# wexiangis/wmix

Measured on AMD Instinct MI355X. Metric: 10 ms frames/s, higher is better.
Workload: dtype f32

## Files before the change

### tools_dev/aec_prof.py

```python
import sys, ctypes; sys.path.insert(0,'.')
import numpy as np, torch
from wmix_amd import synth, _lib
from wmix_amd.aec import AecBatch
dev=torch.device('cuda:0'); S=int(sys.argv[1]) if len(sys.argv)>1 else 65536
import os
if os.environ.get('WMX_TOOL_LIB'): _lib.LIB_PATH=os.environ['WMX_TOOL_LIB']
lib=_lib.lib(); f=lib.wmx_debug_aec_prof; f.argtypes=[ctypes.c_void_p,ctypes.c_int]
ab=AecBatch(S,1,16000,10); nf=24
far=synth.far_end(5,nf,160); near=synth.near_end(50,64,nf,160,far=far)
dfar=torch.from_numpy(far.reshape(nf,160).copy()).to(dev)
dn=torch.from_numpy(np.ascontiguousarray(near.reshape(64,nf,160).transpose(1,0,2))).to(dev).repeat(1,S//64,1).contiguous()
buf=(ctypes.c_ulonglong*16)()
for k in range(nf):
    if k==16: f(buf,1)
    ab.process2_packet_major(dfar[k:k+1],dn[k:k+1])
f(buf,0); v=np.array(buf[:16],dtype=np.float64)
names=['near ring+d,dw fft','dpow+filterfar','y ifft+e,ew fft','scale+adapt','partdelay','xfw+psd','sd/se sums','coh+hNl+scalars','overdrive+cn','ifft+ola','state in','(all pkts)','state out','scale_err','pack','24 ffts']
tot=v[10]+v[12]+v[11]
for n,x in zip(names,v): print('%-20s %8.1f Mcyc %5.1f%%'%(n,x/1e6,100*x/tot))
print('pcm io etc', (v[11]-v[:10].sum()-v[13:].sum())/1e6)
```

### tools_dev/ns_prof.py

```python
import sys, ctypes; sys.path.insert(0,'.')
import numpy as np, torch
from wmix_amd import synth, _lib
from wmix_amd.ns import NsBatch
dev=torch.device('cuda:0'); S=int(sys.argv[1]) if len(sys.argv)>1 else 65536
import os
if os.environ.get('WMX_TOOL_LIB'): _lib.LIB_PATH=os.environ['WMX_TOOL_LIB']
lib=_lib.lib(); f=lib.wmx_debug_ns_prof; f.argtypes=[ctypes.c_void_p,ctypes.c_int]
nb=NsBatch(S,1,16000); nf=int(sys.argv[2]) if len(sys.argv)>2 else 260
x=synth.ns_input(7,64,nf,160)
d=torch.from_numpy(np.ascontiguousarray(x.reshape(64,nf,160).transpose(1,0,2))).to(dev).repeat(1,S//64,1).contiguous()
buf=(ctypes.c_ulonglong*16)()
for k in range(nf):
    if k==nf-8: f(buf,1)
    nb.process_packet_major(d[k:k+1])
f(buf,0); v=np.array(buf[:14],dtype=np.float64)
names=['load+window+energy1','fft fwd','spectrum+log','7 sums','noise est (quantiles)','startup/snr loop','3 sums+flat','lrt loop (log)','ksum+prior+exp loop','noise update+wiener','ifft','td+energy2','synth+hb','output']
for n,x in zip(names,v): print('%-24s %8.1f Mcyc %5.1f%%'%(n,x/1e6,100*x/v.sum()))
```

### wmix_amd/csrc/aec.hip

```cpp
#include <algorithm>
#include <chrono>
#include <cmath>
#include <cstdlib>
#include <cstring>
#include <cstddef>
#include <unordered_map>
#include <vector>
#include "wmx_internal.h"
#include "aec_ctl.h"
#include "cohort_hip.h"
#include "fft_regs.h"
#include "libm_dev.h"

namespace wmx {
namespace {

constexpr int BP = 68;
enum : int {
    AS_W_RE = 0,
    AS_W_IM = AS_W_RE + 12 * BP,
    AS_DPOW = AS_W_IM + 12 * BP,
    AS_DMIN = AS_DPOW + BP,
    AS_DINIT = AS_DMIN + BP,
    AS_SD = AS_DINIT + BP,
// ... 303 lines not shown
    int16_t park[kAecFrame];
#ifdef WMX_AEC_PROF
    unsigned long long prof[16];
#endif
};
#define AEC_ST(x) W.st[(x) - AS_LDS0]

struct AecTaps {
    v2f t[12];
};

__device__ __forceinline__ float uniform_ld(const float *p) {
    return *reinterpret_cast<const float __attribute__((address_space(4))) *>(reinterpret_cast<size_t>(p));
}

typedef const float __attribute__((address_space(1))) *GlobalRow;
__device__ __forceinline__ GlobalRow uniform_row(const float *base, int row, int row_words) {
    const float *p = base + (size_t)row * row_words;
    asm volatile("" : "+s"(p));
    return (GlobalRow)p;
}

__device__ __forceinline__ float row_ld(GlobalRow row, unsigned lane_bytes, int word) {
    return *(GlobalRow)((const char __attribute__((address_space(1))) *)(row + word) + lane_bytes);
}

constexpr int kHistRowBytes = 130 * 4, kHistMid = 2860;
struct HistRows {
    GlobalRow base;
    unsigned voff;
// ... 12 lines not shown

__device__ __forceinline__ int ring_at(int pos, int i) {
    const int t = pos + i;
    return t >= kAecRing ? t - kAecRing : t;
}
__device__ __forceinline__ float *fa_row(AecWaveLds &W, int r) { return &W.fa[0][0] + __umul24((unsigned)r, (unsigned)FAS); }
__device__ __forceinline__ int opaque_lane(int x) {
#ifndef WMX_AEC_HOIST
    asm volatile("" : "+v"(x));
#endif
    __builtin_assume(x >= 0 && x < 64);
    return x;
}

template <int MULT>
__device__ __forceinline__ void aec_block(const AecConstsNear &K, const float *__restrict__ curves_g, const PowTables *__restrict__ powtab, AecWaveLds &W, AecTaps &taps,
                                          const AecFarBufs &F, const AecBlkPlan &bp, const AecNoiseEntry *__restrict__ noise_tab, const int lane_in) {
    int lane = opaque_lane(lane_in);
    int *Si = reinterpret_cast<int *>(W.st) - AS_LDS0;
    const float mu = MULT == 1 ? 0.6f : 0.5f, err_thr = MULT == 1 ? 2e-6f : 1.5e-6f;
    const float scale = 2.0f / 128;
    const int n = bp.hist_n;
    int blk_flags;
    {
        int nctr = __builtin_amdgcn_readfirstlane(Si[AS_NOISECTR]), dctr = __builtin_amdgcn_readfirstlane(Si[AS_DELAYCTR]);
        blk_flags = nctr > 50 ? kAecFlagNoiseMin : 0;
        if (nctr < 500 * MULT) {
            nctr++;
            blk_flags |= kAecFlagNoiseInit;
        }
        dctr++;
        if (dctr == 10 * MULT) dctr = 0;
// ... 359 lines not shown
    const int diverge = ((Si[AS_DIVERGE] ? 1.05f : 1.0f) * seSum > sdSum) ? 1 : 0;
    const bool reset_filter = seSum > (19.95f * sdSum);
    wave_sync();
    if (lane == 0) Si[AS_DIVERGE] = diverge;
    if (reset_filter) {
#pragma unroll
        for (int p = 0; p < 12; p++) {
            taps.t[p] = v2f{0.f, 0.f};
            if (lane == 0) W.wn[p] = 0.f;
        }
    }
    AEC_PROF(6);
    AEC_RELANE();
    const uint32_t nseed = (uint32_t)__builtin_amdgcn_readfirstlane(Si[AS_NSEED]);
    const uint2 *jump = reinterpret_cast<const uint2 *>(noise_tab + kAecNoiseTab);
    const uint2 jl = jump[(lane + 63) & 63], j64 = jump[63];
    const AecNoiseEntry nz = noise_tab[((nseed * jl.x + jl.y) & 0x7FFFFFFFu) >> 16];
    const float nz_c = nz.c, nz_s = nz.s;
    if (lane == 0) Si[AS_NSEED] = (int)((nseed * j64.x + j64.y) & 0x7FFFFFFFu);
    {
        auto coh = [&](int b, float &cde, float &cxd) {
            const float sde_r = AEC_ST(AS_SDE_RE + b), sde_i = AEC_ST(AS_SDE_IM + b), sxd_r = AEC_ST(AS_SXD_RE + b),
                        sxd_i = AEC_ST(AS_SXD_IM + b);
            cde = (sde_r * sde_r + sde_i * sde_i) / (AEC_ST(AS_SD + b) * AEC_ST(AS_SE + b) + 1e-10f);
            cxd = (sxd_r * sxd_r + sxd_i * sxd_i) / (AEC_ST(AS_SX + b) * AEC_ST(AS_SD + b) + 1e-10f);
        };
        float a0, a1, c0, c1;
        coh(lane, a0, a1);
#if !defined(WMX_AEC_EXP) || WMX_AEC_EXP < 1
        coh(kAecPart, c0, c1);
#else
// ... 172 lines not shown
            AEC_ST(AS_OUT_RING + ring_at(bp.out_wr, i + 1)) = o1;
        }
        wave_sync();
        if (lane >= 32) {
            AEC_ST(AS_OUTBUF + i) = pt.x * scale * K.hanning[kAecPart - i];
            AEC_ST(AS_OUTBUF + i + 1) = pt.y * scale * K.hanning[kAecPart - i - 1];
        }
    }
    AEC_ST(AS_DPREV + lane) = W.cur[lane];
    AEC_ST(AS_EPREV + lane) = W.enew[lane];
    wave_sync();
    AEC_PROF(9);
#undef AEC_RELANE
}

template <int MULT>
#ifndef WMX_AEC_WAVES
#define WMX_AEC_WAVES 4
#endif
__global__ __attribute__((amdgpu_waves_per_eu(WMX_AEC_WAVES, WMX_AEC_WAVES))) __launch_bounds__(64 * kAecWavesPerBlock) void aec_near_kernel(float *__restrict__ state, AecFarBufs F_all,
                                                                          const float *__restrict__ consts_g,
                                                                          const AecPlan *__restrict__ plans, int n_packets, int n_classes,
                                                                          const int32_t *__restrict__ plan_of,
                                                                          const AecNoiseEntry *__restrict__ noise_tab,
                                                                          const int16_t *near_pcm, int16_t *out_pcm, int n_streams,
                                                                          long stream_stride, long packet_stride, int chn, int pkg,
                                                                          const int *__restrict__ stream_far, const uint8_t *__restrict__ active,
                                                                          const int *__restrict__ order) {
    __shared__ AecConstsNear K;
    __shared__ AecWaveLds Wv[kAecWavesPerBlock];
    const int lane = threadIdx.x & 63;
    const int wave = __builtin_amdgcn_readfirstlane(threadIdx.x >> 6);
    int sidx;
    if (order) {
        const unsigned i = blockIdx.x, per = gridDim.x >> 3;
        sidx = __builtin_amdgcn_readfirstlane(order[((i & 7u) * per + (i >> 3)) * kAecWavesPerBlock + wave]);
    } else {
        sidx = blockIdx.x * kAecWavesPerBlock + wave;
    }
    const bool live = sidx >= 0 && stream_active(active, sidx, n_streams);
    const int sl = (sidx >= 0 && sidx < n_streams) ? sidx : 0;
    const int grp = stream_far ? __builtin_amdgcn_readfirstlane(stream_far[sl]) : 0;
    const AecFarBufs F = far_group(F_all, grp);
    plans += plan_of ? __builtin_amdgcn_readfirstlane(plan_of[grp]) : grp;
    float *gst = state + (size_t)sl * AS_WORDS;
    constexpr int kConstIt = (kAecConstNearWords + 64 * kAecWavesPerBlock - 1) / (64 * kAecWavesPerBlock);
    float kc[kConstIt];
#pragma unroll
    for (int k = 0; k < kConstIt; k++) {
        const int i = threadIdx.x + 64 * kAecWavesPerBlock * k;
        kc[k] = consts_g[i < kAecConstNearWords ? i : 0];
    }
    int16_t pcm0[2][2];
    {
        const int16_t *in0 = near_pcm + (size_t)sl * stream_stride;
#pragma unroll
        for (int s = 0; s < 2; s++)
#pragma unroll
            for (int h = 0; h < 2; h++) {
                const int i = lane + 64 * h;
                const bool want = i < kAecFrame && s * kAecFrame + i < pkg;
                const int16_t v = in0[want ? (s * kAecFrame + i) * chn : 0];
                pcm0[s][h] = want ? v : (int16_t)0;
            }
    }
    AecTaps taps;
#pragma unroll
    for (int p = 0; p < 12; p++) {
        taps.t[p].x = gst[AS_W_RE + p * BP + lane];
        taps.t[p].y = gst[AS_W_IM + p * BP + lane];
    }
    const float wn0 = gst[AS_W_RE + (lane < 12 ? lane : 0) * BP + kAecPart];
    constexpr int kChunks = (AS_LDS_WORDS / 4 + 63) / 64;
    float4 c[kChunks];
    {
        const float4 *g4 = reinterpret_cast<const float4 *>(gst + AS_LDS0);
#pragma unroll
        for (int k = 0; k < kChunks; k++) {
            const int i = lane + 64 * k;
            c[k] = g4[i < AS_LDS_WORDS / 4 ? i : i - 64];
        }
    }
#pragma unroll
    for (int k = 0; k < kConstIt; k++) {
        const int i = threadIdx.x + 64 * kAecWavesPerBlock * k;
        if (i < kAecConstNearWords) reinterpret_cast<float *>(&K)[i] = kc[k];
    }
    asm volatile("s_waitcnt lgkmcnt(0)\n\ts_barrier" ::: "memory");
    if (!live) return;
    const PowTables *powtab = reinterpret_cast<const PowTables *>(consts_g + kAecConstWords);
    AecWaveLds &W = Wv[wave];
#ifdef WMX_AEC_PROF
    if (lane < 16) W.prof[lane] = 0;
#endif
    AEC_PROF_START;
    if (lane < 12) W.wn[lane] = wn0;
    {
        float4 *s4 = reinterpret_cast<float4 *>(W.st);
#pragma unroll
        for (int k = 0; k < kChunks; k++) {
            const int i = lane + 64 * k;
            s4[i < AS_LDS_WORDS / 4 ? i : i - 64] = c[k];
        }
    }
#pragma unroll
    for (int h = 0; h < 2; h++) {
        const int i = lane + 64 * h;
        if (i < kAecFrame) {
            W.fa[0][i] = (float)pcm0[0][h];
            W.park[i] = pcm0[1][h];
        }
    }
    wave_sync();
    AEC_PROF(10);
    for (int p = 0; p < n_packets; p++) {
        const AecPlan &pl = plans[(size_t)p * n_classes];
        if (!pl.has_near) continue;
        const size_t off = (size_t)sidx * stream_stride + (size_t)p * packet_stride;
        const int16_t *in = near_pcm + off;
        int16_t *out = out_pcm + off;
        if (pl.passthrough) {
            for (int i = lane; i < pkg; i += 64) {
                const int16_t v = in[i * chn];
                for (int c = 0; c < chn; c++) out[i * chn + c] = v;
            }
            continue;
        }
        for (int s = 0; s < pl.n_sub; s++) {
            const AecSubPlan &sp = pl.sub[s];
            const int ln = opaque_lane(lane);
#pragma unroll
            for (int h = 0; h < 2; h++) {
                const int i = ln + 64 * h;
                if (i >= kAecFrame) continue;
                const float v = (p == 0 && s < 2) ? (s == 0 ? W.fa[0][i] : (float)W.park[i]) : (float)in[(s * kAecFrame + i) * chn];
                AEC_ST(AS_NEAR_RING + ring_at(sp.near_wr, i)) = v;
            }
            wave_sync();
            for (int k = 0; k < sp.n_blocks; k++)
                aec_block<MULT>(K, consts_g + kAecConstNearWords, powtab, W, taps, F, pl.blk[sp.first_blk + k], noise_tab, lane);
            for (int i = opaque_lane(lane); i < kAecFrame; i += 64) {
                const int16_t v = (int16_t)AEC_ST(AS_OUT_RING + ring_at(sp.out_rd, i));
                for (int c = 0; c < chn; c++) out[(s * kAecFrame + i) * chn + c] = v;
            }
            wave_sync();
        }
    }
    wave_sync();
    AEC_PROF(11);
    asm volatile("" : "+s"(gst));
    float __attribute__((address_space(1))) *gout = (float __attribute__((address_space(1))) *)gst;
    const int ln = opaque_lane(lane);
#pragma unroll
    for (int p = 0; p < 12; p++) {
        gout[AS_W_RE + p * BP + ln] = taps.t[p].x;
        gout[AS_W_IM + p * BP + ln] = taps.t[p].y;
    }
    if (ln < 12) gout[AS_W_RE + ln * BP + kAecPart] = W.wn[ln];
    {
        typedef float v4f __attribute__((ext_vector_type(4)));
        v4f __attribute__((address_space(1))) *g4 = (v4f __attribute__((address_space(1))) *)(gout + AS_LDS0);
        const v4f *s4 = reinterpret_cast<const v4f *>(W.st);
        for (int i = ln; i < AS_LDS_WORDS / 4; i += 64) g4[i] = s4[i];
    }
    AEC_PROF(12);
#ifdef WMX_AEC_PROF
    if (lane < 16) atomicAdd(&g_aec_prof[lane], W.prof[lane]);
#endif
}
#ifdef WMX_AEC_PROF
extern "C" int wmx_debug_aec_prof(unsigned long long *out16, int reset) {
    hipDeviceSynchronize();
    hipMemcpyFromSymbol(out16, HIP_SYMBOL(g_aec_prof), sizeof(unsigned long long) * 16);
    if (reset) {
        unsigned long long z[16] = {0};
        hipMemcpyToSymbol(HIP_SYMBOL(g_aec_prof), z, sizeof(z));
    }
    return 0;
}
#endif


// ... 82 lines not shown
    wmx::AecFarBufs far;
    int *d_stream_far;
    std::vector<int32_t> h_cohort_of;
    std::vector<int32_t> h_order[2];
    int h_order_sel;
    int32_t *d_order;
    unsigned order_wgs;
    bool order_dirty;
    int order_age;
    static constexpr int kOrderEvery = 16;
    wmx::AecNoiseEntry *d_noise_tab;
    wmx::StreamLife life;
    bool timing;
    std::vector<hipEvent_t> tev;
    size_t tev_used;
    bool no_order;
    double ctl_seconds;
    long ctl_calls;
    static constexpr size_t kMaxTimingEvents = 4 * 4096;
};

extern "C" {

int wmx_aec_destroy(wmx_aec *h) {
    WMX_ON_DEVICE(h);
    if (!h) return 0;
    if (h->d_state) (void)hipFree(h->d_state);
    if (h->d_consts) (void)hipFree(h->d_consts);
    if (h->d_stream_far) (void)hipFree(h->d_stream_far);
    if (h->d_order) (void)hipFree(h->d_order);
// ... 134 lines not shown
    std::vector<float> st(AS_WORDS, 0.f);
    for (int b = 0; b < 65; b++) {
        st[AS_DMIN + b] = 1.0e6f;
        st[AS_SD + b] = 1.f;
        st[AS_SX + b] = 1.f;
    }
    st[AS_HNLFBMIN] = 1.f;
    st[AS_HNLFBLOCALMIN] = 1.f;
    st[AS_HNLXDAVGMIN] = 1.f;
    st[AS_OVERDRIVE] = 2.f;
    st[AS_OVERDRIVESM] = 2.f;
    {
        const uint32_t seed0 = 777u;
        memcpy(&st[AS_NSEED], &seed0, 4);
    }
    WMX_CREATE_TRY(wmx_aec_destroy(h), hipMalloc(&h->d_state, (size_t)AS_WORDS * n_streams * sizeof(float)));
    WMX_CREATE_TRY(wmx_aec_destroy(h), hipMalloc(&h->d_consts, sizeof(K) + sizeof(PowTables)));
    for (hipEvent_t &ev : h->co.plan_free) WMX_CREATE_TRY(wmx_aec_destroy(h), hipEventCreateWithFlags(&ev, hipEventDisableTiming));
    {
        const int rc = h->co.reserve(n_far, [h] { aec_carve_far(h); });
        if (rc != 0) {
            wmx_aec_destroy(h);
            return rc;
        }
    }
    if (n_far > 1) {
        WMX_CREATE_TRY(wmx_aec_destroy(h), hipMalloc(&h->d_stream_far, sizeof(int) * n_streams));
        if (stream_far) {
            WMX_CREATE_TRY(wmx_aec_destroy(h), hipMemcpy(h->d_stream_far, stream_far, sizeof(int) * n_streams, hipMemcpyHostToDevice));
        } else {
// ... 127 lines not shown
            WMX_HIP(hipEventRecord(tv[0], fs));
        }
        hipLaunchKernelGGL(aec_far_kernel, dim3((unsigned)L.G), dim3(64), 0, fs, h->far, h->d_consts, L.dp, L.chunk, L.C, L.plan_of,
                           d_far ? d_far + (size_t)L.done * far_packet_stride : nullptr, far_packet_stride, far_group_stride, h->chn, gpow1np,
                           L.by_value, L.hp[0]);
        WMX_LAUNCH_CHECK();
        if (tv) WMX_HIP(hipEventRecord(tv[1], fs));
        return 0;
    };
    auto near = [&](const CohortLaunch<AecPlan> &L) {
        if (tv) WMX_HIP(hipEventRecord(tv[2], s));
        const int16_t *nin = d_near + (size_t)L.done * packet_stride;
        int16_t *nout = d_out + (size_t)L.done * packet_stride;
        if (h->order_age < wmx_aec::kOrderEvery) h->order_age++;
        const int32_t *order = ordered ? h->d_order : nullptr;
        const unsigned grid = ordered ? h->order_wgs : (unsigned)((h->n_streams + kAecWavesPerBlock - 1) / kAecWavesPerBlock);
        const dim3 blk(64 * kAecWavesPerBlock);
        if (h->freq == 8000)
            hipLaunchKernelGGL((aec_near_kernel<1>), dim3(grid), blk, 0, s, h->d_state, h->far, h->d_consts, L.dp, L.chunk, L.C, L.plan_of,
                               h->d_noise_tab, nin, nout, h->n_streams, stream_stride, packet_stride, h->chn, h->pkg, h->d_stream_far,
                               h->life.d_active, order);
        else
            hipLaunchKernelGGL((aec_near_kernel<2>), dim3(grid), blk, 0, s, h->d_state, h->far, h->d_consts, L.dp, L.chunk, L.C, L.plan_of,
                               h->d_noise_tab, nin, nout, h->n_streams, stream_stride, packet_stride, h->chn, h->pkg, h->d_stream_far,
                               h->life.d_active, order);
        WMX_LAUNCH_CHECK();
        if (tv) WMX_HIP(hipEventRecord(tv[3], s));
        return 0;
    };
    return run_cohorts(h, "wmx_aec_run", mode, d_far, far_packet_stride, far_group_stride, d_near, d_out, n_packets, stream_stride,
                       packet_stride, delay_ms, cohort_on, cohort_rc, s, before, plan, far, near);
}

int wmx_aec_reset_streams(wmx_aec *h, const int32_t *idx, int n, int cohort, void *stream) {
    using namespace wmx;
    int refused = 0;
    if (h && (cohort < -1 || cohort >= h->co.n()))
        refused = WMX_EINVAL;
    else if (h && cohort >= 0 && h->co.n() > 1 && !h->d_stream_far)
        refused = WMX_ESTATE;
// ... 145 lines not shown
```

### wmix_amd/csrc/ns.hip

```cpp
#include <cmath>
#include <vector>
#include "stage_life.h"
#include "fft_ooura.h"
#include "libm_dev.h"
#include "ns_layout.h"

namespace wmx {
namespace {

constexpr int kStartupShort = 50;
constexpr int kStartupLong = 200;
constexpr int kHistBins = 1000;
constexpr int kUpdateWindow = 500;
constexpr int kStartBand = 5;

constexpr int kNsWavesPerBlock = 4;

template <int L>
struct NsConstLds {
    FftTables tab;
    float window[L];
    float logi[NsLayout<L>::MP];
    NsLibmTables lm;
};
// ... 57 lines not shown
        if (i + 1 < MP4) {
            const float4 b = *reinterpret_cast<const float4 *>(mine + 4 * i + 4);
            acc += b.x;
            acc += b.y;
            acc += b.z;
            acc += b.w;
        }
    }
    return acc;
}
__device__ __noinline__ static float tanh_call(float x, const NsLibmTables *m) { return fast_tanh(x, *m); }
__device__ __forceinline__ float lane_value(float v, int k) { return __int_as_float(__builtin_amdgcn_readlane(__float_as_int(v), k)); }

template <int L, int CHN>
__device__ void ns_frame(const NsConstLds<L> &K, NsWaveLds<L> &W, float *__restrict__ st, unsigned short *__restrict__ hist,
                         const int16_t *in, int16_t *out, const int pkg, const int lane_in) {
    using Y = NsLayout<L>;
    constexpr int chn = CHN;
    int lane = lane_in;
#define NS_RELANE() asm volatile("" : "+v"(lane))
    NS_RELANE();
#ifdef WMX_NS_PROF
    long long prof_t0 = clock64();
#endif
    constexpr int M = Y::M, B = Y::B, NT = L / 64, NC = L / 2;
    struct StF {
        GlobalF g;
        unsigned i;
        __device__ __forceinline__ operator float() const { return row_ld(g, i); }
        __device__ __forceinline__ void operator=(float v) const { row_st(g, i, v); }
    };
// ... 36 lines not shown
#else
    constexpr int NI = (M + 63) / 64;
#endif
    float pf_quant[NI], pf_dens[NI][3], pf_lq[NI][3], pf_pause[NI];
#pragma unroll
    for (int k = 0; k < NI; k++) {
        const int b = lane + 64 * k < M ? lane + 64 * k : M - 1;
        pf_pause[k] = ST(Y::MAGN_AVG_PAUSE + b);
        pf_quant[k] = ST(Y::QUANTILE + b);
#pragma unroll
        for (int q = 0; q < 3; q++) {
            pf_dens[k][q] = ST(Y::DENSITY + q * Y::MP + b);
            pf_lq[k][q] = ST(Y::LQUANTILE + q * Y::MP + b);
        }
    }
    wave_sync();
#pragma unroll
    for (int k = 0; k < NT; k++) {
        const int i = lane + 64 * k;
        if (64 * k + 63 < B) continue;
        if (i >= B) {
            ST(Y::IN_BUF + i) = buf[k];
            if (chn == 2) ST(Y::HB_BUF + i) = hb[k];
        }
    }
#pragma unroll
    for (int k = 0; k < NT; k++) {
        const int i = lane + 64 * k;
        const float w = K.window[i] * buf[k];
        W.fa[i] = w;
        tdst[i] = w * w;
    }
    wave_sync();
    const float energy1 = sum_range(tdst, 0, L, lane);
    wave_sync();
    NS_PROF(0);

    float hb_gain = 1.f;
    const bool zero_frame = (energy1 == 0.0f);
    float t_re[(Y::M + 63) / 64], t_im[(Y::M + 63) / 64], t_prev[(Y::M + 63) / 64], t_snrq[(Y::M + 63) / 64];

    if (!zero_frame) {
        const int block_ind = SCI(S_BLOCK_IND) + 1;
        STI(Y::S_BLOCK_IND) = block_ind;
        const int update_flag = SCI(S_UPDATE_FLAG);
        const bool startup = block_ind < kStartupShort;
        const float overdrive = 1.1f, denoise_bound = 0.125f;

        NS_RELANE();
        rdft_forward<NC>(W.fa, &K.tab, lane);
        if (lane < Y::MP - M) W.r0[M + lane] = 0.f;
// ... 457 lines not shown
            ST(Y::MAGN_PREV + b) = mg;
            ST(Y::NOISE_PREV + b) = nz;
            W.snrp[b] = f;
            if (b == 0)
                W.fa[0] = re;
            else if (b == M - 1)
                W.fa[1] = re;
            else {
                W.fa[2 * b] = re;
                W.fa[2 * b + 1] = im;
            }
        }
        wave_sync();
        NS_PROF(9);
        NS_RELANE();
        rdft_inverse<NC>(W.fa, &K.tab, lane);
        NS_PROF(10);
        float td[NT];
#pragma unroll
        for (int k = 0; k < NT; k++) {
            const int i = lane + 64 * k;
            td[k] = W.fa[i] * (2.f / L);
            tdst[i] = td[k] * td[k];
        }
        wave_sync();
        NS_PROF(11);
        float factor = 1.f;
        if (block_ind > kStartupLong) {
            const float energy2 = sum_range(tdst, 0, L, lane);
            float gain = sqrtf(energy2 / (energy1 + 1.f));
// ... 59 lines not shown

#ifndef WMX_NS_W128
#define WMX_NS_W128 7
#endif
#ifndef WMX_NS_W256
#define WMX_NS_W256 5
#endif
template <int L>
struct NsOcc {
    static constexpr int kWaves = L == 128 ? WMX_NS_W128 : WMX_NS_W256;
};
template <int L, int CHN>
__global__ __launch_bounds__(64 * kNsWavesPerBlock) __attribute__((amdgpu_waves_per_eu(NsOcc<L>::kWaves, NsOcc<L>::kWaves))) void ns_kernel(float *__restrict__ state, unsigned short *__restrict__ hists,
                                                                      const float *__restrict__ consts, const int16_t *in, int16_t *out,
                                                                      int n_streams, int n_packets, long stream_stride,
                                                                      long packet_stride, int pkg, const uint8_t *__restrict__ active) {
    using Y = NsLayout<L>;
    __shared__ NsConstLds<L> K;
    __shared__ NsWaveLds<L> Wv[kNsWavesPerBlock];
    {
        float *dst = reinterpret_cast<float *>(&K);
        constexpr int NCONST = sizeof(NsConstLds<L>) / 4, NIT = (NCONST + 64 * kNsWavesPerBlock - 1) / (64 * kNsWavesPerBlock);
        float c[NIT];
#pragma unroll
        for (int k = 0; k < NIT; k++) {
            const int i = threadIdx.x + 64 * kNsWavesPerBlock * k;
            c[k] = consts[i < NCONST ? i : 0];
        }
#pragma unroll
        for (int k = 0; k < NIT; k++) {
            const int i = threadIdx.x + 64 * kNsWavesPerBlock * k;
            if (i < NCONST) dst[i] = c[k];
        }
    }
    __syncthreads();
    const int lane = threadIdx.x & 63;
    const int wave = __builtin_amdgcn_readfirstlane(threadIdx.x >> 6);
    const int sidx = blockIdx.x * kNsWavesPerBlock + wave;
    if (!stream_active(active, sidx, n_streams)) return;
    float *st = state + (size_t)sidx * Y::WORDS;
    unsigned short *hist = hists + (size_t)sidx * 3 * kHistBins;
    {
        float *wb = Wv[wave].magn;
        constexpr int NARR = 9;
        if (lane < NARR * (Y::MP - Y::M)) wb[(lane / (Y::MP - Y::M)) * Y::MP + Y::M + lane % (Y::MP - Y::M)] = 0.f;
    }
#ifdef WMX_NS_PROF
    if (lane < 16) Wv[wave].prof[lane] = 0;
#endif
    for (int p = 0; p < n_packets; p++) {
        const size_t off = (size_t)sidx * stream_stride + (size_t)p * packet_stride;
        ns_frame<L, CHN>(K, Wv[wave], st, hist, in + off, out + off, pkg, lane);
    }
#ifdef WMX_NS_PROF
    if (lane < 16) atomicAdd(&g_ns_prof[lane], Wv[wave].prof[lane]);
#endif
}
#ifdef WMX_NS_PROF
extern "C" int wmx_debug_ns_prof(unsigned long long *out16, int reset) {
    (void)hipDeviceSynchronize();
    (void)hipMemcpyFromSymbol(out16, HIP_SYMBOL(g_ns_prof), sizeof(unsigned long long) * 16);
    if (reset) {
        unsigned long long z[16] = {0};
        (void)hipMemcpyToSymbol(HIP_SYMBOL(g_ns_prof), z, sizeof(z));
    }
    return 0;
}
#endif

}
}

struct wmx_ns {
    int device;
    int n_streams, chn, freq, L, pkg;
    float *d_state;
    unsigned short *d_hist;
    float *d_consts;
    float *d_tmpl;
    size_t words;
    wmx::StreamLife life;
};

namespace {

template <int L>
void build_ns_template(std::vector<float> &st, std::vector<float> &consts) {
    using Y = wmx::NsLayout<L>;
    st.assign(Y::WORDS, 0.f);
    int *sti = reinterpret_cast<int *>(st.data());
    for (int q = 0; q < 3; q++)
        for (int b = 0; b < Y::M; b++) {
            st[Y::LQUANTILE + q * Y::MP + b] = 8.f;
            st[Y::DENSITY + q * Y::MP + b] = 0.3f;
        }
// ... 63 lines not shown
    if ((h->device = wmx::current_device()) < 0) {
        delete h;
        return WMX_ENODEV;
    }
    h->n_streams = n_streams;
    h->chn = chn;
    h->freq = freq;
    h->L = (freq == 8000) ? 128 : 256;
    h->pkg = freq / 1000 * 10;
    std::vector<float> st, consts;
    if (h->L == 128)
        build_ns_template<128>(st, consts);
    else
        build_ns_template<256>(st, consts);
    h->words = st.size();
    WMX_CREATE_TRY(wmx_ns_destroy(h), hipMalloc(&h->d_state, h->words * sizeof(float) * (size_t)n_streams));
    WMX_CREATE_TRY(wmx_ns_destroy(h), hipMalloc(&h->d_hist, (size_t)n_streams * 3 * 1000 * sizeof(unsigned short)));
    WMX_CREATE_TRY(wmx_ns_destroy(h), hipMalloc(&h->d_consts, consts.size() * sizeof(float)));
    WMX_CREATE_TRY(wmx_ns_destroy(h), hipMalloc(&h->d_tmpl, st.size() * sizeof(float)));
    WMX_CREATE_TRY(wmx_ns_destroy(h), hipMemcpy(h->d_consts, consts.data(), consts.size() * sizeof(float), hipMemcpyHostToDevice));
    WMX_CREATE_TRY(wmx_ns_destroy(h), hipMemcpy(h->d_tmpl, st.data(), st.size() * sizeof(float), hipMemcpyHostToDevice));
    WMX_CREATE_TRY(wmx_ns_destroy(h), hipMemset(h->d_hist, 0, (size_t)n_streams * 3 * 1000 * sizeof(unsigned short)));
    hipLaunchKernelGGL(ns_fill_state, dim3(1024), dim3(256), 0, nullptr, h->d_state, h->d_tmpl, (int)h->words, n_streams);
    WMX_CREATE_TRY(wmx_ns_destroy(h), hipGetLastError());
    WMX_CREATE_TRY(wmx_ns_destroy(h), hipDeviceSynchronize());
    *out = h;
    return 0;
}

int wmx_ns_destroy(wmx_ns *h) {
// ... 46 lines not shown
    WMX_ON_DEVICE(h);
    if (!h || n_packets < 0) {
        wmx::set_error("wmx_ns_process: bad argument");
        return WMX_EINVAL;
    }
    if (n_packets == 0) return 0;
    if (!d_in || !d_out) {
        wmx::set_error("wmx_ns_process: null buffer");
        return WMX_EINVAL;
    }
    const int per_pkt = h->pkg * h->chn;
    if (packet_stride < per_pkt || (h->n_streams > 1 && stream_stride < per_pkt)) {
        wmx::set_error("wmx_ns_process: strides (%ld, %ld) smaller than a packet (%d samples)", stream_stride, packet_stride, per_pkt);
        return WMX_EINVAL;
    }
    const unsigned grid = (unsigned)((h->n_streams + wmx::kNsWavesPerBlock - 1) / wmx::kNsWavesPerBlock);
    hipStream_t s = wmx::as_stream(stream);
#define NS_LAUNCH(LL, CC)                                                                                                  \
    hipLaunchKernelGGL((wmx::ns_kernel<LL, CC>), dim3(grid), dim3(64 * wmx::kNsWavesPerBlock), 0, s, h->d_state, h->d_hist, \
                       h->d_consts, d_in, d_out, h->n_streams, n_packets, stream_stride, packet_stride, h->pkg, h->life.d_active)
    if (h->L == 128) {
        if (h->chn == 1)
            NS_LAUNCH(128, 1);
        else
            NS_LAUNCH(128, 2);
    } else {
        if (h->chn == 1)
            NS_LAUNCH(256, 1);
        else
            NS_LAUNCH(256, 2);
    }
#undef NS_LAUNCH
    WMX_LAUNCH_CHECK();
    return 0;
}
// ... 39 lines not shown
```

### wmix_amd/csrc/wmx_internal.h

```cpp
#pragma once
#include <hip/hip_runtime.h>
#include <cstdarg>
#include <cstdint>
#include <cstdio>
#include <cstring>
#include <vector>
#include "../../include/wmix_amd.h"
#include "build_flags.h"

#ifdef WMX_FAULT_INJECTION
namespace wmx {
hipError_t fault_point();
}
#define WMX_FAULT_OR(expr) (wmx::fault_point() != hipSuccess ? hipErrorUnknown : (expr))
#else
#define WMX_FAULT_OR(expr) (expr)
#endif

#define WMX_HIP(expr)                                                         \
    do {                                                                      \
        hipError_t _e = WMX_FAULT_OR(expr);                                   \
        if (_e != hipSuccess) return wmx::hip_fail(_e, #expr, __FILE__, __LINE__); \
    } while (0)

// ... 168 lines not shown
__device__ __forceinline__ void row_st(GlobalF row, unsigned idx, float v) {
    *(GlobalF)((char __attribute__((address_space(1))) *)row + 4u * idx) = v;
}

template <class T>
__global__ void fill_rows_idx(T *state, const T *tmpl, int words, const int32_t *idx, int n_idx) {
    for (int j = blockIdx.x; j < n_idx; j += gridDim.x) {
        T *dst = state + (size_t)idx[j] * words;
        for (int i = threadIdx.x; i < words; i += blockDim.x) dst[i] = tmpl ? tmpl[i] : T(0);
    }
}
__device__ __forceinline__ bool stream_active(const uint8_t *active, int sidx, int n_streams) {
    return sidx < n_streams && (!active || active[sidx] != 0);
}
__device__ __forceinline__ void touch_done(int &sink) { asm volatile("s_waitcnt vmcnt(0)" : "+v"(sink) : : "memory"); }
#endif

}

#define WMX_LAUNCH_CHECK() WMX_HIP(hipGetLastError())

#define WMX_ON_DEVICE(h)                              \
    wmx::DeviceScope _dev_scope((h) ? (h)->device : -1); \
    WMX_HIP(_dev_scope.err)
```

Measured before the change: 60.17 million.

## Make AEC and NS kernels persistent with grid-stride slots over streams

The AEC and NS kernels now launch at most an occupancy-derived number of workgroups and loop over stream slots with a grid stride, instead of launching one workgroup per slot. The per-block constant LDS load and barrier run only on the first visit, and the AEC kernel reads its arguments and plan structures through the constant (scalar) address space. The aim is to amortise workgroup launch and constant-setup cost. The trade-off is that load balance now depends on the static slot assignment. Optional touch-ahead prefetch of the next stream's state is added behind macros, and the profiling scripts gain extra counters.

```diff
diff --git a/tools_dev/aec_prof.py b/tools_dev/aec_prof.py
--- a/tools_dev/aec_prof.py
+++ b/tools_dev/aec_prof.py
@@ -15,7 +15,7 @@
     if k==16: f(buf,1)
     ab.process2_packet_major(dfar[k:k+1],dn[k:k+1])
 f(buf,0); v=np.array(buf[:16],dtype=np.float64)
-names=['near ring+d,dw fft','dpow+filterfar','y ifft+e,ew fft','scale+adapt','partdelay','xfw+psd','sd/se sums','coh+hNl+scalars','overdrive+cn','ifft+ola','state in','(all pkts)','state out','scale_err','pack','24 ffts']
-tot=v[10]+v[12]+v[11]
+names=['near ring+d,dw fft','dpow+filterfar','y ifft+e,ew fft','scale+adapt','partdelay','xfw+psd','sd/se sums','coh+hNl+scalars','overdrive+cn','ifft+ola','state in','(all pkts)','state out','entry..constants barrier','-','-']
+tot=v[10]+v[12]+v[11]+v[13]
 for n,x in zip(names,v): print('%-20s %8.1f Mcyc %5.1f%%'%(n,x/1e6,100*x/tot))
-print('pcm io etc', (v[11]-v[:10].sum()-v[13:].sum())/1e6)
+print('pcm io etc', (v[11]-v[:10].sum())/1e6)
diff --git a/tools_dev/ns_prof.py b/tools_dev/ns_prof.py
--- a/tools_dev/ns_prof.py
+++ b/tools_dev/ns_prof.py
@@ -13,6 +13,6 @@
 for k in range(nf):
     if k==nf-8: f(buf,1)
     nb.process_packet_major(d[k:k+1])
-f(buf,0); v=np.array(buf[:14],dtype=np.float64)
-names=['load+window+energy1','fft fwd','spectrum+log','7 sums','noise est (quantiles)','startup/snr loop','3 sums+flat','lrt loop (log)','ksum+prior+exp loop','noise update+wiener','ifft','td+energy2','synth+hb','output']
+f(buf,0); v=np.array(buf[:16],dtype=np.float64)
+names=['window+energy1','fft fwd','spectrum+log','7 sums','noise est (quantiles)','startup/snr loop','3 sums+flat','lrt loop (log)','ksum+prior+exp loop','noise update+wiener','ifft','td+energy2','synth+hb','output','frame loads landed','entry..constants barrier']
 for n,x in zip(names,v): print('%-24s %8.1f Mcyc %5.1f%%'%(n,x/1e6,100*x/v.sum()))
diff --git a/wmix_amd/csrc/aec.hip b/wmix_amd/csrc/aec.hip
--- a/wmix_amd/csrc/aec.hip
+++ b/wmix_amd/csrc/aec.hip
@@ -341,6 +341,13 @@
     return *reinterpret_cast<const float __attribute__((address_space(4))) *>(reinterpret_cast<size_t>(p));
 }
 
+template <class T>
+using LaunchConst = const T __attribute__((address_space(4)));
+template <class T>
+__device__ __forceinline__ LaunchConst<T> *launch_const(const T *p) {
+    return reinterpret_cast<LaunchConst<T> *>(reinterpret_cast<size_t>(p));
+}
+
 typedef const float __attribute__((address_space(1))) *GlobalRow;
 __device__ __forceinline__ GlobalRow uniform_row(const float *base, int row, int row_words) {
     const float *p = base + (size_t)row * row_words;
@@ -383,8 +390,8 @@
 }
 
 template <int MULT>
-__device__ __forceinline__ void aec_block(const AecConstsNear &K, const float *__restrict__ curves_g, const PowTables *__restrict__ powtab, AecWaveLds &W, AecTaps &taps,
-                                          const AecFarBufs &F, const AecBlkPlan &bp, const AecNoiseEntry *__restrict__ noise_tab, const int lane_in) {
+__device__ __forceinline__ void aec_block(const AecConstsNear &K, LaunchConst<float> *curves_g, const PowTables *__restrict__ powtab, AecWaveLds &W, AecTaps &taps,
+                                          const AecFarBufs &F, LaunchConst<AecBlkPlan> &bp, const AecNoiseEntry *__restrict__ noise_tab, const int lane_in) {
     int lane = opaque_lane(lane_in);
     int *Si = reinterpret_cast<int *>(W.st) - AS_LDS0;
     const float mu = MULT == 1 ? 0.6f : 0.5f, err_thr = MULT == 1 ? 2e-6f : 1.5e-6f;
@@ -774,7 +781,8 @@
     AEC_RELANE();
     const uint32_t nseed = (uint32_t)__builtin_amdgcn_readfirstlane(Si[AS_NSEED]);
     const uint2 *jump = reinterpret_cast<const uint2 *>(noise_tab + kAecNoiseTab);
-    const uint2 jl = jump[(lane + 63) & 63], j64 = jump[63];
+    const uint2 jl = jump[(lane + 63) & 63];
+    const uint2 j64 = make_uint2(launch_const(&jump[63].x)[0], launch_const(&jump[63].y)[0]);
     const AecNoiseEntry nz = noise_tab[((nseed * jl.x + jl.y) & 0x7FFFFFFFu) >> 16];
     const float nz_c = nz.c, nz_s = nz.s;
     if (lane == 0) Si[AS_NSEED] = (int)((nseed * j64.x + j64.y) & 0x7FFFFFFFu);
@@ -977,42 +985,56 @@
 #undef AEC_RELANE
 }
 
+struct AecNearArgs {
+    float *state;
+    AecFarBufs F_all;
+    const float *consts_g;
+    const AecPlan *plans;
+    int n_packets, n_classes;
+    const int32_t *plan_of;
+    const AecNoiseEntry *noise_tab;
+    const int16_t *near_pcm;
+    int16_t *out_pcm;
+    int n_streams;
+    long stream_stride, packet_stride;
+    int chn, pkg;
+    const int *stream_far;
+    const uint8_t *active;
+    const int *order;
+    int n_slots;
+};
 template <int MULT>
-#ifndef WMX_AEC_WAVES
-#define WMX_AEC_WAVES 4
-#endif
-__global__ __attribute__((amdgpu_waves_per_eu(WMX_AEC_WAVES, WMX_AEC_WAVES))) __launch_bounds__(64 * kAecWavesPerBlock) void aec_near_kernel(float *__restrict__ state, AecFarBufs F_all,
-                                                                          const float *__restrict__ consts_g,
-                                                                          const AecPlan *__restrict__ plans, int n_packets, int n_classes,
-                                                                          const int32_t *__restrict__ plan_of,
-                                                                          const AecNoiseEntry *__restrict__ noise_tab,
-                                                                          const int16_t *near_pcm, int16_t *out_pcm, int n_streams,
-                                                                          long stream_stride, long packet_stride, int chn, int pkg,
-                                                                          const int *__restrict__ stream_far, const uint8_t *__restrict__ active,
-                                                                          const int *__restrict__ order) {
-    __shared__ AecConstsNear K;
-    __shared__ AecWaveLds Wv[kAecWavesPerBlock];
-    const int lane = threadIdx.x & 63;
-    const int wave = __builtin_amdgcn_readfirstlane(threadIdx.x >> 6);
+__device__ __forceinline__ void aec_near_visit(AecConstsNear &K, AecWaveLds &W, const unsigned slot, const int wave, const bool first, const long long t_entry,
+                                               float *__restrict__ state, const AecFarBufs &F_all, const float *__restrict__ consts_g,
+                                               const AecPlan *__restrict__ plans, int n_packets, int n_classes, const int32_t *__restrict__ plan_of,
+                                               const AecNoiseEntry *__restrict__ noise_tab, const int16_t *near_pcm, int16_t *out_pcm, int n_streams,
+                                               long stream_stride, long packet_stride, int chn, int pkg, const int *__restrict__ stream_far,
+                                               const uint8_t *__restrict__ active, const int *__restrict__ order, int n_slots) {
+    const PowTables *powtab = reinterpret_cast<const PowTables *>(consts_g + kAecConstWords);
+    const int lane = opaque_lane((int)(threadIdx.x & 63));
     int sidx;
     if (order) {
-        const unsigned i = blockIdx.x, per = gridDim.x >> 3;
-        sidx = __builtin_amdgcn_readfirstlane(order[((i & 7u) * per + (i >> 3)) * kAecWavesPerBlock + wave]);
+        const unsigned per = (unsigned)n_slots >> 3;
+        sidx = launch_const(order)[((slot & 7u) * per + (slot >> 3)) * kAecWavesPerBlock + wave];
     } else {
-        sidx = blockIdx.x * kAecWavesPerBlock + wave;
+        sidx = (int)slot * kAecWavesPerBlock + wave;
     }
     const bool live = sidx >= 0 && stream_active(active, sidx, n_streams);
+    if (!live && !first) return;
+    AEC_PROF_START;
     const int sl = (sidx >= 0 && sidx < n_streams) ? sidx : 0;
-    const int grp = stream_far ? __builtin_amdgcn_readfirstlane(stream_far[sl]) : 0;
+    const int grp = stream_far ? launch_const(stream_far)[sl] : 0;
     const AecFarBufs F = far_group(F_all, grp);
-    plans += plan_of ? __builtin_amdgcn_readfirstlane(plan_of[grp]) : grp;
+    LaunchConst<AecPlan> *vplans = launch_const(plans) + (plan_of ? launch_const(plan_of)[grp] : grp);
     float *gst = state + (size_t)sl * AS_WORDS;
     constexpr int kConstIt = (kAecConstNearWords + 64 * kAecWavesPerBlock - 1) / (64 * kAecWavesPerBlock);
     float kc[kConstIt];
-#pragma unroll
-    for (int k = 0; k < kConstIt; k++) {
-        const int i = threadIdx.x + 64 * kAecWavesPerBlock * k;
-        kc[k] = consts_g[i < kAecConstNearWords ? i : 0];
+    if (first) {
+#pragma unroll
+        for (int k = 0; k < kConstIt; k++) {
+            const int i = threadIdx.x + 64 * kAecWavesPerBlock * k;
+            kc[k] = consts_g[i < kAecConstNearWords ? i : 0];
+        }
     }
     int16_t pcm0[2][2];
     {
@@ -1035,31 +1057,32 @@
     }
     const float wn0 = gst[AS_W_RE + (lane < 12 ? lane : 0) * BP + kAecPart];
     constexpr int kChunks = (AS_LDS_WORDS / 4 + 63) / 64;
-    float4 c[kChunks];
-    {
-        const float4 *g4 = reinterpret_cast<const float4 *>(gst + AS_LDS0);
+    typedef float v4f __attribute__((ext_vector_type(4)));
+    v4f c[kChunks];
+    {
+        const v4f *g4 = reinterpret_cast<const v4f *>(gst + AS_LDS0);
 #pragma unroll
         for (int k = 0; k < kChunks; k++) {
             const int i = lane + 64 * k;
             c[k] = g4[i < AS_LDS_WORDS / 4 ? i : i - 64];
         }
     }
-#pragma unroll
-    for (int k = 0; k < kConstIt; k++) {
-        const int i = threadIdx.x + 64 * kAecWavesPerBlock * k;
-        if (i < kAecConstNearWords) reinterpret_cast<float *>(&K)[i] = kc[k];
-    }
-    asm volatile("s_waitcnt lgkmcnt(0)\n\ts_barrier" ::: "memory");
-    if (!live) return;
-    const PowTables *powtab = reinterpret_cast<const PowTables *>(consts_g + kAecConstWords);
-    AecWaveLds &W = Wv[wave];
+    if (first) {
+#pragma unroll
+        for (int k = 0; k < kConstIt; k++) {
+            const int i = threadIdx.x + 64 * kAecWavesPerBlock * k;
+            if (i < kAecConstNearWords) reinterpret_cast<float *>(&K)[i] = kc[k];
+        }
+        asm volatile("s_waitcnt lgkmcnt(0)\n\ts_barrier" ::: "memory");
 #ifdef WMX_AEC_PROF
-    if (lane < 16) W.prof[lane] = 0;
-#endif
-    AEC_PROF_START;
+        t_prev = clock64();
+        if (lane == 0) W.prof[13] += (unsigned long long)(t_prev - t_entry);
+#endif
+        if (!live) return;
+    }
     if (lane < 12) W.wn[lane] = wn0;
     {
-        float4 *s4 = reinterpret_cast<float4 *>(W.st);
+        v4f *s4 = reinterpret_cast<v4f *>(W.st);
 #pragma unroll
         for (int k = 0; k < kChunks; k++) {
             const int i = lane + 64 * k;
@@ -1076,8 +1099,11 @@
     }
     wave_sync();
     AEC_PROF(10);
+#ifdef WMX_AEC_TOUCH_AHEAD
+    int sink = 0;
+#endif
     for (int p = 0; p < n_packets; p++) {
-        const AecPlan &pl = plans[(size_t)p * n_classes];
+        LaunchConst<AecPlan> &pl = vplans[(size_t)p * n_classes];
         if (!pl.has_near) continue;
         const size_t off = (size_t)sidx * stream_stride + (size_t)p * packet_stride;
         const int16_t *in = near_pcm + off;
@@ -1090,7 +1116,7 @@
             continue;
         }
         for (int s = 0; s < pl.n_sub; s++) {
-            const AecSubPlan &sp = pl.sub[s];
+            LaunchConst<AecSubPlan> &sp = pl.sub[s];
             const int ln = opaque_lane(lane);
 #pragma unroll
             for (int h = 0; h < 2; h++) {
@@ -1100,8 +1126,27 @@
                 AEC_ST(AS_NEAR_RING + ring_at(sp.near_wr, i)) = v;
             }
             wave_sync();
+#ifdef WMX_AEC_TOUCH_AHEAD
+            if (p == n_packets - 1 && s == pl.n_sub - 1 && sp.n_blocks > 0 && slot + gridDim.x < (unsigned)n_slots) {
+                const unsigned nslot = slot + gridDim.x;
+                const int nidx = order ? launch_const(order)[((nslot & 7u) * ((unsigned)n_slots >> 3) + (nslot >> 3)) * kAecWavesPerBlock + wave]
+                                       : (int)nslot * kAecWavesPerBlock + wave;
+                if (nidx >= 0 && nidx < n_streams) {
+                    const unsigned l128 = 128u * (unsigned)opaque_lane(lane), last = (unsigned)AS_WORDS * 4u - 1u;
+                    const char *nst = reinterpret_cast<const char *>(state + (size_t)nidx * AS_WORDS);
+                    const char *npk = reinterpret_cast<const char *>(near_pcm + (size_t)nidx * stream_stride);
+                    const unsigned plast = (unsigned)(pkg * chn) * 2u - 1u;
+                    touch_line(nst + (l128 < last ? l128 : last), sink);
+                    touch_line(nst + (l128 + 8192u < last ? l128 + 8192u : last), sink);
+                    touch_line(npk + (l128 < plast ? l128 : plast), sink);
+                }
+            }
+#endif
             for (int k = 0; k < sp.n_blocks; k++)
-                aec_block<MULT>(K, consts_g + kAecConstNearWords, powtab, W, taps, F, pl.blk[sp.first_blk + k], noise_tab, lane);
+                aec_block<MULT>(K, launch_const(consts_g + kAecConstNearWords), powtab, W, taps, F, pl.blk[sp.first_blk + k], noise_tab, lane);
+#ifdef WMX_AEC_TOUCH_AHEAD
+            asm volatile("" : "+v"(sink));
+#endif
             for (int i = opaque_lane(lane); i < kAecFrame; i += 64) {
                 const int16_t v = (int16_t)AEC_ST(AS_OUT_RING + ring_at(sp.out_rd, i));
                 for (int c = 0; c < chn; c++) out[(s * kAecFrame + i) * chn + c] = v;
@@ -1121,14 +1166,49 @@
     }
     if (ln < 12) gout[AS_W_RE + ln * BP + kAecPart] = W.wn[ln];
     {
-        typedef float v4f __attribute__((ext_vector_type(4)));
         v4f __attribute__((address_space(1))) *g4 = (v4f __attribute__((address_space(1))) *)(gout + AS_LDS0);
         const v4f *s4 = reinterpret_cast<const v4f *>(W.st);
         for (int i = ln; i < AS_LDS_WORDS / 4; i += 64) g4[i] = s4[i];
     }
     AEC_PROF(12);
+}
+
+template <int MULT>
+#ifndef WMX_AEC_WAVES
+#define WMX_AEC_WAVES 4
+#endif
+__global__ __attribute__((amdgpu_waves_per_eu(WMX_AEC_WAVES, WMX_AEC_WAVES))) __launch_bounds__(64 * kAecWavesPerBlock) void aec_near_kernel(const AecNearArgs args_by_value) {
+    __shared__ AecConstsNear K;
+    __shared__ AecWaveLds Wv[kAecWavesPerBlock];
 #ifdef WMX_AEC_PROF
-    if (lane < 16) atomicAdd(&g_aec_prof[lane], W.prof[lane]);
+    const long long t_entry = clock64();
+#else
+    const long long t_entry = 0;
+#endif
+    const int wave = __builtin_amdgcn_readfirstlane(threadIdx.x >> 6);
+    AecWaveLds &W = Wv[wave];
+#ifdef WMX_AEC_PROF
+    if ((threadIdx.x & 63) < 16) W.prof[threadIdx.x & 63] = 0;
+#endif
+    (void)args_by_value;
+#ifdef WMX_AEC_STAGGER
+    for (unsigned i = (unsigned)__builtin_amdgcn_s_getreg((3 << 11) | 4) & 3u; i > 0; i--) __builtin_amdgcn_s_sleep(WMX_AEC_STAGGER);
+#endif
+    typedef const AecNearArgs __attribute__((address_space(4))) *NearArgs;
+    NearArgs ap = (NearArgs)__builtin_amdgcn_kernarg_segment_ptr();
+    for (unsigned slot = blockIdx.x;; slot += gridDim.x) {
+        asm volatile("" : "+s"(ap));
+        const int n_slots = ap->n_slots;
+        if (slot >= (unsigned)n_slots) break;
+        aec_near_visit<MULT>(K, W, slot, wave, slot == blockIdx.x, t_entry, ap->state,
+                             AecFarBufs{ap->F_all.pre, ap->F_all.tring, ap->F_all.hist, ap->F_all.nyq, ap->F_all.hist_w, ap->F_all.xpow_seq,
+                                        ap->F_all.xpow, ap->F_all.group_words},
+                             ap->consts_g, ap->plans, ap->n_packets, ap->n_classes, ap->plan_of, ap->noise_tab, ap->near_pcm, ap->out_pcm,
+                             ap->n_streams, ap->stream_stride, ap->packet_stride, ap->chn, ap->pkg, ap->stream_far, ap->active, ap->order, n_slots);
+    }
+#ifdef WMX_AEC_PROF
+    wave_sync();
+    if ((threadIdx.x & 63) < 16) atomicAdd(&g_aec_prof[threadIdx.x & 63], W.prof[threadIdx.x & 63]);
 #endif
 }
 #ifdef WMX_AEC_PROF
@@ -1241,6 +1321,7 @@
     bool timing;
     std::vector<hipEvent_t> tev;
     size_t tev_used;
+    unsigned persist_wgs;
     bool no_order;
     double ctl_seconds;
     long ctl_calls;
@@ -1405,6 +1486,8 @@
         const uint32_t seed0 = 777u;
         memcpy(&st[AS_NSEED], &seed0, 4);
     }
+    WMX_CREATE_TRY(wmx_aec_destroy(h), freq == 8000 ? persistent_wgs(aec_near_kernel<1>, 64 * kAecWavesPerBlock, h->device, &h->persist_wgs)
+                                                    : persistent_wgs(aec_near_kernel<2>, 64 * kAecWavesPerBlock, h->device, &h->persist_wgs));
     WMX_CREATE_TRY(wmx_aec_destroy(h), hipMalloc(&h->d_state, (size_t)AS_WORDS * n_streams * sizeof(float)));
     WMX_CREATE_TRY(wmx_aec_destroy(h), hipMalloc(&h->d_consts, sizeof(K) + sizeof(PowTables)));
     for (hipEvent_t &ev : h->co.plan_free) WMX_CREATE_TRY(wmx_aec_destroy(h), hipEventCreateWithFlags(&ev, hipEventDisableTiming));
@@ -1562,16 +1645,16 @@
         int16_t *nout = d_out + (size_t)L.done * packet_stride;
         if (h->order_age < wmx_aec::kOrderEvery) h->order_age++;
         const int32_t *order = ordered ? h->d_order : nullptr;
-        const unsigned grid = ordered ? h->order_wgs : (unsigned)((h->n_streams + kAecWavesPerBlock - 1) / kAecWavesPerBlock);
+        const unsigned slots = ordered ? h->order_wgs : (unsigned)((h->n_streams + kAecWavesPerBlock - 1) / kAecWavesPerBlock);
+        unsigned grid = std::min(slots, h->persist_wgs);
+        if (ordered && grid > 8u) grid &= ~7u;
         const dim3 blk(64 * kAecWavesPerBlock);
+        const AecNearArgs args{h->d_state, h->far, h->d_consts, L.dp, L.chunk, L.C, L.plan_of, h->d_noise_tab, nin, nout, h->n_streams, stream_stride,
+                               packet_stride, h->chn, h->pkg, h->d_stream_far, h->life.d_active, order, (int)slots};
         if (h->freq == 8000)
-            hipLaunchKernelGGL((aec_near_kernel<1>), dim3(grid), blk, 0, s, h->d_state, h->far, h->d_consts, L.dp, L.chunk, L.C, L.plan_of,
-                               h->d_noise_tab, nin, nout, h->n_streams, stream_stride, packet_stride, h->chn, h->pkg, h->d_stream_far,
-                               h->life.d_active, order);
+            hipLaunchKernelGGL((aec_near_kernel<1>), dim3(grid), blk, 0, s, args);
         else
-            hipLaunchKernelGGL((aec_near_kernel<2>), dim3(grid), blk, 0, s, h->d_state, h->far, h->d_consts, L.dp, L.chunk, L.C, L.plan_of,
-                               h->d_noise_tab, nin, nout, h->n_streams, stream_stride, packet_stride, h->chn, h->pkg, h->d_stream_far,
-                               h->life.d_active, order);
+            hipLaunchKernelGGL((aec_near_kernel<2>), dim3(grid), blk, 0, s, args);
         WMX_LAUNCH_CHECK();
         if (tv) WMX_HIP(hipEventRecord(tv[3], s));
         return 0;
diff --git a/wmix_amd/csrc/ns.hip b/wmix_amd/csrc/ns.hip
--- a/wmix_amd/csrc/ns.hip
+++ b/wmix_amd/csrc/ns.hip
@@ -1,3 +1,4 @@
+#include <algorithm>
 #include <cmath>
 #include <vector>
 #include "stage_life.h"
@@ -95,7 +96,11 @@
 
 template <int L, int CHN>
 __device__ void ns_frame(const NsConstLds<L> &K, NsWaveLds<L> &W, float *__restrict__ st, unsigned short *__restrict__ hist,
-                         const int16_t *in, int16_t *out, const int pkg, const int lane_in) {
+                         const int16_t *in, int16_t *out, const int pkg, const int lane_in
+#ifdef WMX_NS_TOUCH_AHEAD
+                         , int &sink, const char *next_st, const char *next_in
+#endif
+) {
     using Y = NsLayout<L>;
     constexpr int chn = CHN;
     int lane = lane_in;
@@ -162,6 +167,10 @@
             pf_lq[k][q] = ST(Y::LQUANTILE + q * Y::MP + b);
         }
     }
+#ifdef WMX_NS_PROF
+    asm volatile("s_waitcnt vmcnt(0)" ::: "memory");
+    NS_PROF(14);
+#endif
     wave_sync();
 #pragma unroll
     for (int k = 0; k < NT; k++) {
@@ -183,6 +192,9 @@
     const float energy1 = sum_range(tdst, 0, L, lane);
     wave_sync();
     NS_PROF(0);
+#ifdef WMX_NS_TOUCH_AHEAD
+    asm volatile("" : "+v"(sink));
+#endif
 
     float hb_gain = 1.f;
     const bool zero_frame = (energy1 == 0.0f);
@@ -670,6 +682,17 @@
         wave_sync();
         NS_PROF(9);
         NS_RELANE();
+#ifdef WMX_NS_TOUCH_AHEAD
+        if (next_st) {
+            const unsigned l128 = 128u * (unsigned)lane, last = (unsigned)Y::WORDS * 4u - 1u;
+            unsigned a = l128 < last ? l128 : last, b = l128 + 8192u < last ? l128 + 8192u : last;
+            if (chn == 1 && a >= (unsigned)Y::HB_BUF * 4u && a + 128u <= (unsigned)Y::DENSITY * 4u) a = 0;
+            touch_line(next_st + a, sink);
+            if (last >= 8192u) touch_line(next_st + b, sink);
+            const unsigned plast = (unsigned)(pkg * chn) * 2u - 1u;
+            touch_line(next_in + (l128 < plast ? l128 : plast), sink);
+        }
+#endif
         rdft_inverse<NC>(W.fa, &K.tab, lane);
         NS_PROF(10);
         float td[NT];
@@ -759,10 +782,13 @@
 __global__ __launch_bounds__(64 * kNsWavesPerBlock) __attribute__((amdgpu_waves_per_eu(NsOcc<L>::kWaves, NsOcc<L>::kWaves))) void ns_kernel(float *__restrict__ state, unsigned short *__restrict__ hists,
                                                                       const float *__restrict__ consts, const int16_t *in, int16_t *out,
                                                                       int n_streams, int n_packets, long stream_stride,
-                                                                      long packet_stride, int pkg, const uint8_t *__restrict__ active) {
+                                                                      long packet_stride, int pkg, const uint8_t *__restrict__ active, int n_slots) {
     using Y = NsLayout<L>;
     __shared__ NsConstLds<L> K;
     __shared__ NsWaveLds<L> Wv[kNsWavesPerBlock];
+#ifdef WMX_NS_PROF
+    const long long t_entry = clock64();
+#endif
     {
         float *dst = reinterpret_cast<float *>(&K);
         constexpr int NCONST = sizeof(NsConstLds<L>) / 4, NIT = (NCONST + 64 * kNsWavesPerBlock - 1) / (64 * kNsWavesPerBlock);
@@ -781,10 +807,6 @@
     __syncthreads();
     const int lane = threadIdx.x & 63;
     const int wave = __builtin_amdgcn_readfirstlane(threadIdx.x >> 6);
-    const int sidx = blockIdx.x * kNsWavesPerBlock + wave;
-    if (!stream_active(active, sidx, n_streams)) return;
-    float *st = state + (size_t)sidx * Y::WORDS;
-    unsigned short *hist = hists + (size_t)sidx * 3 * kHistBins;
     {
         float *wb = Wv[wave].magn;
         constexpr int NARR = 9;
@@ -792,10 +814,28 @@
     }
 #ifdef WMX_NS_PROF
     if (lane < 16) Wv[wave].prof[lane] = 0;
-#endif
-    for (int p = 0; p < n_packets; p++) {
-        const size_t off = (size_t)sidx * stream_stride + (size_t)p * packet_stride;
-        ns_frame<L, CHN>(K, Wv[wave], st, hist, in + off, out + off, pkg, lane);
+    if (lane == 0) Wv[wave].prof[15] = (unsigned long long)(clock64() - t_entry);
+#endif
+#ifdef WMX_NS_TOUCH_AHEAD
+    int sink = 0;
+#endif
+    for (unsigned slot = blockIdx.x; slot < (unsigned)n_slots; slot += gridDim.x) {
+        const int sidx = (int)slot * kNsWavesPerBlock + wave;
+        if (!stream_active(active, sidx, n_streams)) continue;
+        float *st = state + (size_t)sidx * Y::WORDS;
+        unsigned short *hist = hists + (size_t)sidx * 3 * kHistBins;
+        for (int p = 0; p < n_packets; p++) {
+            const size_t off = (size_t)sidx * stream_stride + (size_t)p * packet_stride;
+#ifdef WMX_NS_TOUCH_AHEAD
+            const int nidx = (int)(slot + gridDim.x) * kNsWavesPerBlock + wave;
+            const bool ahead = p == n_packets - 1 && slot + gridDim.x < (unsigned)n_slots && nidx < n_streams;
+            ns_frame<L, CHN>(K, Wv[wave], st, hist, in + off, out + off, pkg, lane, sink,
+                             ahead ? reinterpret_cast<const char *>(state + (size_t)nidx * Y::WORDS) : nullptr,
+                             reinterpret_cast<const char *>(in + (size_t)(ahead ? nidx : sidx) * stream_stride));
+#else
+            ns_frame<L, CHN>(K, Wv[wave], st, hist, in + off, out + off, pkg, lane);
+#endif
+        }
     }
 #ifdef WMX_NS_PROF
     if (lane < 16) atomicAdd(&g_ns_prof[lane], Wv[wave].prof[lane]);
@@ -824,6 +864,7 @@
     float *d_consts;
     float *d_tmpl;
     size_t words;
+    unsigned persist_wgs;
     wmx::StreamLife life;
 };
 
@@ -917,6 +958,13 @@
     else
         build_ns_template<256>(st, consts);
     h->words = st.size();
+    {
+        const int blk = 64 * wmx::kNsWavesPerBlock;
+        WMX_CREATE_TRY(wmx_ns_destroy(h), h->L == 128 ? (chn == 1 ? wmx::persistent_wgs(wmx::ns_kernel<128, 1>, blk, h->device, &h->persist_wgs)
+                                                                  : wmx::persistent_wgs(wmx::ns_kernel<128, 2>, blk, h->device, &h->persist_wgs))
+                                                      : (chn == 1 ? wmx::persistent_wgs(wmx::ns_kernel<256, 1>, blk, h->device, &h->persist_wgs)
+                                                                  : wmx::persistent_wgs(wmx::ns_kernel<256, 2>, blk, h->device, &h->persist_wgs)));
+    }
     WMX_CREATE_TRY(wmx_ns_destroy(h), hipMalloc(&h->d_state, h->words * sizeof(float) * (size_t)n_streams));
     WMX_CREATE_TRY(wmx_ns_destroy(h), hipMalloc(&h->d_hist, (size_t)n_streams * 3 * 1000 * sizeof(unsigned short)));
     WMX_CREATE_TRY(wmx_ns_destroy(h), hipMalloc(&h->d_consts, consts.size() * sizeof(float)));
@@ -993,11 +1041,12 @@
         wmx::set_error("wmx_ns_process: strides (%ld, %ld) smaller than a packet (%d samples)", stream_stride, packet_stride, per_pkt);
         return WMX_EINVAL;
     }
-    const unsigned grid = (unsigned)((h->n_streams + wmx::kNsWavesPerBlock - 1) / wmx::kNsWavesPerBlock);
+    const unsigned slots = (unsigned)((h->n_streams + wmx::kNsWavesPerBlock - 1) / wmx::kNsWavesPerBlock);
+    const unsigned grid = std::min(slots, h->persist_wgs);
     hipStream_t s = wmx::as_stream(stream);
 #define NS_LAUNCH(LL, CC)                                                                                                  \
     hipLaunchKernelGGL((wmx::ns_kernel<LL, CC>), dim3(grid), dim3(64 * wmx::kNsWavesPerBlock), 0, s, h->d_state, h->d_hist, \
-                       h->d_consts, d_in, d_out, h->n_streams, n_packets, stream_stride, packet_stride, h->pkg, h->life.d_active)
+                       h->d_consts, d_in, d_out, h->n_streams, n_packets, stream_stride, packet_stride, h->pkg, h->life.d_active, (int)slots)
     if (h->L == 128) {
         if (h->chn == 1)
             NS_LAUNCH(128, 1);
diff --git a/wmix_amd/csrc/wmx_internal.h b/wmix_amd/csrc/wmx_internal.h
--- a/wmix_amd/csrc/wmx_internal.h
+++ b/wmix_amd/csrc/wmx_internal.h
@@ -3,6 +3,7 @@
 #include <cstdarg>
 #include <cstdint>
 #include <cstdio>
+#include <cstdlib>
 #include <cstring>
 #include <vector>
 #include "../../include/wmix_amd.h"
@@ -206,6 +207,22 @@
     return sidx < n_streams && (!active || active[sidx] != 0);
 }
 __device__ __forceinline__ void touch_done(int &sink) { asm volatile("s_waitcnt vmcnt(0)" : "+v"(sink) : : "memory"); }
+
+template <class Kernel>
+inline hipError_t persistent_wgs(Kernel kernel, int block_threads, int device, unsigned *wgs) {
+    int per_cu = 0, cus = 0;
+    hipError_t e = hipOccupancyMaxActiveBlocksPerMultiprocessor(&per_cu, kernel, block_threads, 0);
+    if (e == hipSuccess) e = hipDeviceGetAttribute(&cus, hipDeviceAttributeMultiprocessorCount, device);
+    if (e != hipSuccess) return e;
+    if (per_cu < 1 || cus < 1) return hipErrorLaunchOutOfResources;
+    unsigned n = (unsigned)per_cu * (unsigned)cus;
+    if (const char *cap = getenv("WMIX_AMD_PERSIST_WGS")) {
+        const long v = strtol(cap, nullptr, 10);
+        if (v >= 1 && (unsigned long)v < n) n = (unsigned)v;
+    }
+    *wgs = n;
+    return hipSuccess;
+}
 #endif
 
 }
```

After: 54.24 million. 0.901x the previous value.
